# hi-paris/Prosody-Control-French-TTS

Hardware: AMD Instinct MI355X
Metric: audio-seconds/sec prosody+align throughput, 16 kHz French (higher is better)
Workload: dtype fp16-resid16 (MFMA legs) + f64 (F0 / LUFS)

## Files before the change

prosody-control-french-tts_amd/csrc/pce_ctx.hip:

```cpp
#include "pce_internal.h"
#include <cstdlib>
#include <cstring>
#include <cstdarg>

int pce_fail(pce_ctx *ctx, int code, const char *fmt, ...)
{
    char buf[512];
    va_list ap; va_start(ap, fmt);
    vsnprintf(buf, sizeof buf, fmt, ap);
    va_end(ap);
    if (ctx) ctx->err = buf;
    return code;
}

KernelTimer::KernelTimer(pce_ctx *ctx, int kid, hipStream_t on, double work_flops) : c(ctx), id(kid), s(on ? on : ctx->stream), flops(work_flops)
{
    if (!c->prof) return;
    auto take = [&]() -> hipEvent_t {
        if (!c->ev_pool.empty()) { hipEvent_t e = c->ev_pool.back(); c->ev_pool.pop_back(); return e; }
        hipEvent_t e = nullptr;
        if (hipEventCreate(&e) != hipSuccess) return nullptr;
        return e;
    };
    a = take(); b = take();
// ... 73 lines not shown
        return nullptr;
    }
    if (device < 0 || device >= n) {
        if (err && errlen) snprintf(err, errlen, "device %d out of range (0..%d)", device, n - 1);
        return nullptr;
    }
    if ((e = hipSetDevice(device)) != hipSuccess) return fail("hipSetDevice", e);
    hipDeviceProp_t prop;
    if ((e = hipGetDeviceProperties(&prop, device)) != hipSuccess) return fail("hipGetDeviceProperties", e);
    pce_ctx *c = new (std::nothrow) pce_ctx();
    if (!c) { if (err && errlen) snprintf(err, errlen, "out of host memory"); return nullptr; }
    c->device = device;
    c->cu_count = prop.multiProcessorCount;
    if (stream) { c->stream = (hipStream_t)stream; c->own_stream = false; }
    else {
        if ((e = hipStreamCreateWithFlags(&c->stream, hipStreamNonBlocking)) != hipSuccess) { delete c; return fail("hipStreamCreate", e); }
        c->own_stream = true;
    }
    c->no_side = getenv("PCE_NO_AUX") != nullptr;
    c->stft_two_fft = getenv("PCE_STFT_TWO_FFT") != nullptr;
    c->generic_median = getenv("PCE_ALIGN_GENERIC_MEDIAN") != nullptr;
    c->gemm_flat = !(getenv("PCE_GEMM_FLAT") && atoi(getenv("PCE_GEMM_FLAT")) == 0);
    if (const char *re = getenv("PCE_RESID_EPILOGUE")) c->resid_epilogue = atoi(re) == 0 ? 0 : atoi(re) == 2 ? 2 : 1;
    c->en_cpb = getenv("PCE_EN_CPB") ? atoi(getenv("PCE_EN_CPB")) : 0;
    c->gemm_skinny = !(getenv("PCE_GEMM_SKINNY") && atoi(getenv("PCE_GEMM_SKINNY")) == 0);
    c->self_rows = !(getenv("PCE_SELF_ROWS") && atoi(getenv("PCE_SELF_ROWS")) == 0);
    c->xattn_absorb = !(getenv("PCE_XATTN_ABSORB") && atoi(getenv("PCE_XATTN_ABSORB")) == 0);
    {
        const char *ops = getenv("PCE_WHISPER_OPERANDS");
        if (ops && *ops && strcmp(ops, "bf16") && strcmp(ops, "fp16") && strcmp(ops, "fp16-resid16")) {
            if (err && errlen) snprintf(err, errlen, "PCE_WHISPER_OPERANDS=%s: bf16, fp16 or fp16-resid16", ops);
            if (c->own_stream) (void)hipStreamDestroy(c->stream);
            delete c;
            return nullptr;
        }
        c->whisper_ops = (ops && !strcmp(ops, "bf16")) ? 0 : (ops && !strcmp(ops, "fp16")) ? 1 : 2;
        c->resid16 = c->whisper_ops == 2;
    }
    c->pitch_refine_praat = getenv("PCE_PITCH_REFINE") && !strcmp(getenv("PCE_PITCH_REFINE"), "praat");
    if (getenv("PCE_DTW_TRACE_MB") && atoll(getenv("PCE_DTW_TRACE_MB")) > 0) c->dtw_trace_budget = (size_t)atoll(getenv("PCE_DTW_TRACE_MB")) << 20;
    int prio_least = 0, prio_greatest = 0;
    (void)hipDeviceGetStreamPriorityRange(&prio_least, &prio_greatest);
    for (int si = 0; si < pce_ctx::SIDE_COUNT; si++) {
        pce_ctx::Side &sd = c->side[si];
        const int prio = si == pce_ctx::SIDE_STFT ? prio_least : 0;
        if ((e = hipStreamCreateWithPriority(&sd.s, hipStreamNonBlocking, prio)) != hipSuccess) { delete c; return fail("hipStreamCreate", e); }
// ... 204 lines not shown
```

prosody-control-french-tts_amd/csrc/pce_internal.h:

```cpp
#pragma once
#include <hip/hip_runtime.h>
#include <cstdint>
#include <cstdio>
#include <cstring>
#include <string>
#include <vector>
#include "pce.h"

#if defined(__HIP_DEVICE_COMPILE__)
#define PCE_NO_PK_F32 __attribute__((target("no-packed-fp32-ops")))
#else
#define PCE_NO_PK_F32
#endif

struct DevBuf {
    void *p = nullptr;
    size_t cap = 0;
    DevBuf() = default;
    DevBuf(const DevBuf &) = delete;
    DevBuf &operator=(const DevBuf &) = delete;
    DevBuf &operator=(DevBuf &&o) noexcept {
        if (this != &o) { release(); p = o.p; cap = o.cap; o.p = nullptr; o.cap = 0; }
        return *this;
    }
// ... 14 lines not shown
struct SliceCache {
    std::vector<pce_slice> v;
    bool valid = false;
    bool same(const pce_slice *s, int32_t n) const {
        return valid && (size_t)n == v.size() && (n == 0 || memcmp(v.data(), s, sizeof(pce_slice) * (size_t)n) == 0);
    }
    void store(const pce_slice *s, int32_t n) { v.assign(s, s + n); valid = true; }
    void drop() { valid = false; v.clear(); }
};

struct pce_ctx {
    int device = 0;
    hipStream_t stream = nullptr;
    bool own_stream = false;
    enum { SIDE_TAIL = 0, SIDE_LUFS = 1, SIDE_STFT = 2, SIDE_COUNT = 3 };
    struct Side { hipStream_t s = nullptr; hipEvent_t fork = nullptr, join = nullptr; bool pending = false; } side[SIDE_COUNT];
    bool no_side = false;
    bool generic_median = false;
    bool pitch_refine_praat = false;
    bool gemm_few_rows = false;
    bool gemm_skinny = true;
    bool gemm_flat = true;
    int resid_epilogue = 1;
    bool stft_two_fft = false;
    std::string err;
    int cu_count = 0;

    DevBuf pcm_own;
    const int16_t *d_pcm = nullptr;
    DevBuf d_clip_off;
    std::vector<int64_t> clip_off;
    int32_t n_clips = 0;
    int32_t rate = 0;

    int en_cpb = 0;
    DevBuf en_work, en_out;
    SliceCache en_cache;
    int64_t en_n_work = 0;
    int32_t en_n = -1;

    DevBuf lu_meta, lu_chunks, lu_blocks, lu_pow, lu_state_end, lu_state_init, lu_energy, lu_zbuf, lu_out, lu_en_work, lu_en_acc;
    SliceCache lu_cache;
    int64_t lu_n_chunks = 0, lu_n_blocks = 0, lu_n_energy_work = 0;
    double lu_coef[13] = {0};
    int32_t lu_n = -1;
    int32_t lu_meter_rate = 0;
// ... 116 lines not shown
```

prosody-control-french-tts_amd/csrc/pce_whisper_impl.inc:

```
#include "pce_internal.h"
#include "pce_wave.h"
#include <algorithm>
#include <cmath>
#include <cstdlib>
#include <type_traits>

#define pce_logmel_run PCE_WFN(pce_logmel_run)
#define pce_logmel_run_at PCE_WFN(pce_logmel_run_at)
#define pce_logmel_fetch PCE_WFN(pce_logmel_fetch)
#define pce_whisper_load PCE_WFN(pce_whisper_load)
#define pce_whisper_encode_run PCE_WFN(pce_whisper_encode_run)
#define pce_whisper_encode_fetch PCE_WFN(pce_whisper_encode_fetch)
#define pce_selftest_attention PCE_WFN(pce_selftest_attention)
#define pce_selftest_attention_ragged PCE_WFN(pce_selftest_attention_ragged)
#define pce_selftest_attn1 PCE_WFN(pce_selftest_attn1)
#define pce_selftest_gemm PCE_WFN(pce_selftest_gemm)
#define pce_selftest_gemm_resid PCE_WFN(pce_selftest_gemm_resid)
#define pce_whisper_decoder_load PCE_WFN(pce_whisper_decoder_load)
#define pce_whisper_align_run PCE_WFN(pce_whisper_align_run)
#define pce_whisper_align_fetch PCE_WFN(pce_whisper_align_fetch)
#define pce_whisper_align_shape PCE_WFN(pce_whisper_align_shape)
#define pce_whisper_align_paths_enqueue PCE_WFN(pce_whisper_align_paths_enqueue)
#define pce_whisper_align_paths_wait PCE_WFN(pce_whisper_align_paths_wait)
#define pce_whisper_sample_keys PCE_WFN(pce_whisper_sample_keys)
// ... 12 lines not shown
                                          const uint8_t *vocab_mask, const pce_whisper_decode_opts *opts, int32_t *next_tokens,
                                          float *next_logprobs, float *probe_prob);
void pce_whisper_free(pce_ctx *c);

namespace {

typedef PCE_OP_T op_t;
typedef __attribute__((ext_vector_type(8))) op_t opx8;
typedef __attribute__((ext_vector_type(4))) float f32x4;

template <class T> struct MfmaOf;
template <> struct MfmaOf<__bf16> {
    typedef __attribute__((ext_vector_type(8))) __bf16 v8;
    static __device__ __forceinline__ f32x4 m16(v8 a, v8 b, f32x4 c) { return __builtin_amdgcn_mfma_f32_16x16x32_bf16(a, b, c, 0, 0, 0); }
};
template <> struct MfmaOf<_Float16> {
    typedef __attribute__((ext_vector_type(8))) _Float16 v8;
    static __device__ __forceinline__ f32x4 m16(v8 a, v8 b, f32x4 c) { return __builtin_amdgcn_mfma_f32_16x16x32_f16(a, b, c, 0, 0, 0); }
};
__device__ __forceinline__ f32x4 mfma16(opx8 a, opx8 b, f32x4 c) { return MfmaOf<op_t>::m16(a, b, c); }

constexpr int W_NFFT = 400, W_HOP = 160, W_BINS = 201, W_FRAMES = 3000, W_SAMPLES = 480000;
constexpr int W_CTX = 1500;
constexpr double W_PI = 3.14159265358979323846;

struct MelTables {
    const float2 *w16;
    const float2 *w400;
    const float2 *w25;
    const float *window;
    const int *mel_lo;
    const int *mel_n;
    const int *mel_off;
    const float *mel_w;
    int mel_total;
};

__device__ __forceinline__ unsigned int f32_order_key(float f)
{
    const unsigned int b = __float_as_uint(f);
    return (b & 0x80000000u) ? ~b : (b | 0x80000000u);
}
__device__ __forceinline__ float f32_from_key(unsigned int k)
{
    return __uint_as_float((k & 0x80000000u) ? (k & 0x7FFFFFFFu) : ~k);
}
// ... 93 lines not shown
                ob[b * (LM_G + 1) + j] = lg;
                vmax = fmaxf(vmax, lg);
            }
        }
        __builtin_amdgcn_fence(__ATOMIC_ACQ_REL, "wavefront"); __builtin_amdgcn_wave_barrier();
      }
      __builtin_amdgcn_fence(__ATOMIC_ACQ_REL, "wavefront"); __builtin_amdgcn_wave_barrier();
      if (!scan && (f_begin + gi * LM_G) * W_HOP - W_NFFT / 2 < len) {
          const int64_t f0 = gi * LM_G;
          const int nj = (int)min<int64_t>(LM_G, n_fr - f0);
          for (int idx = lane; idx < n_mels * LM_G; idx += 64) {
              const int b = idx / LM_G, j = idx - b * LM_G;
              if (j < nj) logspec[((int64_t)clip * n_mels + b) * W_FRAMES + f0 + j] = ob[b * (LM_G + 1) + j];
          }
      }
      __builtin_amdgcn_fence(__ATOMIC_ACQ_REL, "wavefront"); __builtin_amdgcn_wave_barrier();
    }
    vmax = wave_xor_max(vmax);
    if (lane == 0) atomicMax(clip_max + clip, f32_order_key(vmax));
}

__global__ __launch_bounds__(256) void k_logmel_norm(const float *__restrict__ logspec, const unsigned int *__restrict__ clip_max, int n_mels,
                                                    const int64_t *__restrict__ clip_off, const int64_t *__restrict__ frame0, int clip0,
                                                    op_t *__restrict__ out_tm, float *__restrict__ out_f32)
{
    __shared__ float tile[64][65];
    const int clip = clip0 + blockIdx.z, f0 = blockIdx.x * 64, b0 = blockIdx.y * 64;
    const float floor_v = f32_from_key(clip_max[clip]) - 8.0f;
    const int64_t full = clip_off[clip + 1] - clip_off[clip];
    const int64_t len = frame0 ? full : min<int64_t>(full, (int64_t)W_SAMPLES), f_begin = frame0 ? frame0[clip] : 0;
    const float pad_v = (fmaxf(log10f(fmaxf(0.f, 1e-10f)), floor_v) + 4.0f) / 4.0f;
    const int tx = threadIdx.x & 63, ty = threadIdx.x >> 6;
    const bool padded = (f_begin + f0 + tx) * W_HOP - W_NFFT / 2 >= len;
    for (int r = ty; r < 64; r += 4) {
        const int b = b0 + r, f = f0 + tx;
        if (b < n_mels && f < W_FRAMES) {
            const float v = padded ? pad_v : (fmaxf(logspec[((int64_t)clip * n_mels + b) * W_FRAMES + f], floor_v) + 4.0f) / 4.0f;
            if (out_f32) out_f32[(int64_t)b * W_FRAMES + f] = v;
            tile[r][tx] = v;
        }
    }
    if (!out_tm) return;
    __syncthreads();
    for (int r = ty; r < 64; r += 4) {
        const int f = f0 + r, b = b0 + tx;
        if (b < n_mels && f < W_FRAMES) out_tm[((int64_t)clip * (W_FRAMES + 2) + f + 1) * n_mels + b] = (op_t)tile[tx][r];
    }
}

enum { EPI_BF16 = 0, EPI_GELU_BF16 = 1, EPI_GELU_POS_F32 = 2, EPI_RESID_F32 = 3, EPI_QKV = 4, EPI_F32 = 5 };
constexpr int AT_SP = 1536;
constexpr int G_BM = 128, G_BN = 128, G_BK = 64;

constexpr float GELU_C = 0.70710678118654752440f * 1.2011224087864498f;
constexpr float GELU_P = 0.3275911f / 1.2011224087864498f;
__device__ __forceinline__ float gelu_exact(float x)
{
    const float zp = fabsf(x) * GELU_C;
    const float t = __builtin_amdgcn_rcpf(fmaf(zp, GELU_P, 1.0f));
    const float e = __builtin_amdgcn_exp2f(zp * -zp);
    const float poly = fmaf(t, fmaf(t, fmaf(t, fmaf(t, 1.061405429f, -1.453152027f), 1.421413741f), -0.284496736f), 0.254829592f);
    const float erf_abs = fmaf(-(t * poly), e, 1.0f);
    const float h = 0.5f * x;
    return fmaf(fabsf(h), erf_abs, h);
}
__device__ __forceinline__ void gelu_exact8(float (&x)[8])
{
    float zp[8], t[8], e[8], poly[8], h[8];
#pragma unroll
    for (int i = 0; i < 8; i++) zp[i] = fabsf(x[i]) * GELU_C;
#pragma unroll
    for (int i = 0; i < 8; i++) t[i] = __builtin_amdgcn_rcpf(fmaf(zp[i], GELU_P, 1.0f));
#pragma unroll
    for (int i = 0; i < 8; i++) e[i] = __builtin_amdgcn_exp2f(zp[i] * -zp[i]);
#pragma unroll
// ... 26 lines not shown
        const int r0 = wv * 16 + i * 8;
        const int row = r0 + (lane >> 3);
        const int c = swz_chunk(row, lane & 7);
        int gr = row0 + row; if (gr > row_max) gr = row_max;
        const op_t *src = G + (int64_t)gr * ld + k0 + c * 8;
        __builtin_amdgcn_global_load_lds((const __attribute__((address_space(1))) void *)src,
                                         (__attribute__((address_space(3))) void *)(lds_tile + r0 * G_BK), 16, 0, 0);
    }
}

template <int EPI>
__device__ __forceinline__ void gemm_fetch_bias(const float *__restrict__ bias, int n0, int tid, float (&bv)[8], float &bv_col)
{
    constexpr bool OUT_BF16 = (EPI == EPI_BF16 || EPI == EPI_GELU_BF16 || EPI == EPI_QKV);
    const int cx0 = OUT_BF16 ? (tid & 15) * 8 : (tid & 31) * 4;
#pragma unroll
    for (int e = 0; e < 8; e++) bv[e] = (bias && e < (OUT_BF16 ? 8 : 4)) ? bias[n0 + cx0 + e] : 0.f;
    bv_col = (EPI == EPI_QKV && bias) ? bias[n0 + (tid & 127)] : 0.f;
}

template <int EPI>
__device__ __forceinline__ void gemm_store_tile(const float *tile, int tid, int m0, int n0, int M, int N, const float (&bv)[8], float bv_col,
                                                void *__restrict__ Cv, int64_t ldc, int64_t cbase, const float *__restrict__ pos, int pos_T,
                                                int v_col0, int vt_sp)
{
    if (EPI == EPI_QKV && n0 >= v_col0) {
        op_t *vt = reinterpret_cast<op_t *>(const_cast<float *>(pos));
        const int dmodel = N - v_col0, S = pos_T;
        const int cc = tid & 127, rg = tid >> 7;
        const int n = n0 + cc - v_col0, head = n >> 6, dd = n & 63;
        const float bv = bv_col;
#pragma unroll
        for (int p = 0; p < 4; p++) {
            const int row = rg * 8 + 32 * p;
#pragma unroll
            for (int hf = 0; hf < 2; hf++) {
                const int m = m0 + row + 4 * hf;
                if (m >= M) continue;
                const int clip = m / S, t = m - clip * S;
                typedef __attribute__((ext_vector_type(4))) op_t opx4;
                opx4 o;
#pragma unroll
                for (int e = 0; e < 4; e++) o[e] = (op_t)(tile[(row + 4 * hf + e) * G_TLD + cc] + bv);
                *reinterpret_cast<opx4 *>(vt + (((int64_t)clip * (dmodel >> 6) + head) * 64 + dd) * vt_sp + t) = o;
            }
        }
    } else if (EPI == EPI_BF16 || EPI == EPI_GELU_BF16 || EPI == EPI_QKV) {
// ... 12 lines not shown
                o[e] = (op_t)(EPI == EPI_GELU_BF16 ? gelu_exact(t) : t);
            }
            __builtin_nontemporal_store(o, reinterpret_cast<opx8 *>(reinterpret_cast<op_t *>(Cv) + cbase + (int64_t)(m0 + row) * ldc + n0 + cx));
        }
    } else {
        const int cx = (tid & 31) * 4, ry = tid >> 5;
        float4 oldv[8];
        if (EPI == EPI_RESID_F32) {
#pragma unroll
            for (int p = 0; p < 8; p++) {
                const int row = ry + 16 * p;
                oldv[p] = m0 + row < M ? *reinterpret_cast<const float4 *>(reinterpret_cast<const float *>(Cv) + cbase + (int64_t)(m0 + row) * ldc + n0 + cx)
                                       : make_float4(0.f, 0.f, 0.f, 0.f);
            }
        }
#pragma unroll
        for (int p = 0; p < 8; p++) {
            const int row = ry + 16 * p;
            if (m0 + row >= M) continue;
            const float4 v = *reinterpret_cast<const float4 *>(&tile[row * G_TLD + cx]);
            float4 *dst = reinterpret_cast<float4 *>(reinterpret_cast<float *>(Cv) + cbase + (int64_t)(m0 + row) * ldc + n0 + cx);
            float4 o;
            if (EPI == EPI_GELU_POS_F32) {
                const float4 pe = *reinterpret_cast<const float4 *>(pos + (int64_t)((m0 + row) % pos_T) * N + n0 + cx);
                o = make_float4(gelu_exact(v.x + bv[0]) + pe.x, gelu_exact(v.y + bv[1]) + pe.y, gelu_exact(v.z + bv[2]) + pe.z,
                                gelu_exact(v.w + bv[3]) + pe.w);
            } else {
                const float4 old = EPI == EPI_RESID_F32 ? oldv[p] : make_float4(0.f, 0.f, 0.f, 0.f);
                o = make_float4(old.x + v.x + bv[0], old.y + v.y + bv[1], old.z + v.z + bv[2], old.w + v.w + bv[3]);
            }
            *dst = o;
        }
    }
}

template <int EPI, int G_STAGES = 2>
__global__ __launch_bounds__(G_THREADS, G_STAGES == 2 ? 4 : 2) void k_gemm_bf16(const op_t *__restrict__ A, int64_t lda, int64_t a_batch,
                                                        const op_t *__restrict__ B, int M, int N, int K,
                                                        const float *__restrict__ bias, void *__restrict__ Cv, int64_t ldc, int64_t c_batch,
                                                        const float *__restrict__ pos, int pos_T, int v_col0, int vt_sp, int sn_tiles, int sm_tiles)
{
    constexpr int SMEM_ELEMS = (G_STAGES * 2 * G_BM * G_BK * 2 > G_BM * G_TLD * 4 ? G_STAGES * 2 * G_BM * G_BK : G_BM * G_TLD * 2);
    __shared__ __attribute__((aligned(1024))) op_t smem[SMEM_ELEMS];
    const int tid = threadIdx.x, lane = tid & 63, wv = tid >> 6;
    const int wr = wv >> 2, wc = wv & 3;
    const int tiles_n = (int)gridDim.x, tiles_m_pad = (int)gridDim.y;
    int lin = (int)blockIdx.y * tiles_n + (int)blockIdx.x;
    const int total = tiles_n * tiles_m_pad;
    if ((total & 7) == 0) lin = (lin & 7) * (total >> 3) + (lin >> 3);
    int m0, n0;
    {
        const int per = sm_tiles * sn_tiles, sup = lin / per, r = lin - sup * per;
        const int n_sn = tiles_n / sn_tiles;
        const int tm = (sup / n_sn) * sm_tiles + r / sn_tiles, tn = (sup % n_sn) * sn_tiles + r % sn_tiles;
        m0 = tm * G_BM; n0 = tn * G_BN;
        if (m0 >= M) return;
    }
    float bv[8]; float bv_col;
    gemm_fetch_bias<EPI>(bias, n0, tid, bv, bv_col);
    A += (int64_t)blockIdx.z * a_batch;
    f32x4 acc[4][2];
#pragma unroll
    for (int i = 0; i < 4; i++)
#pragma unroll
        for (int j = 0; j < 2; j++) acc[i][j] = f32x4{0.f, 0.f, 0.f, 0.f};
    const int fr = lane & 15, fq = lane >> 4;
    const int nk = K / G_BK;
    constexpr int STAGE = 2 * G_BM * G_BK;
#pragma unroll
    for (int t = 0; t < G_STAGES - 1; t++) {
        const int tt = t < nk ? t : nk - 1;
        stage_tile(A, lda, m0, M - 1, tt * G_BK, smem + t * STAGE, wv, lane);
        stage_tile(B, K, n0, N - 1, tt * G_BK, smem + t * STAGE + G_BM * G_BK, wv, lane);
    }
    for (int kt = 0; kt < nk; kt++) {
        const op_t *sA = smem + (kt % G_STAGES) * STAGE, *sB = sA + G_BM * G_BK;
        __builtin_amdgcn_s_waitcnt(0x0F70 | (((4 * (G_STAGES - 2)) >> 4) << 14) | ((4 * (G_STAGES - 2)) & 15));
        __builtin_amdgcn_s_barrier();
        if (G_STAGES > 2 || kt + G_STAGES - 1 < nk) {
// ... 12 lines not shown
            }
#pragma unroll
            for (int j = 0; j < 2; j++) {
                const int row = wc * 32 + j * 16 + fr;
                b[j] = *reinterpret_cast<const opx8 *>(&sB[row * G_BK + swz_chunk(row, (kk >> 3) + fq) * 8]);
            }
#pragma unroll
            for (int i = 0; i < 4; i++)
#pragma unroll
                for (int j = 0; j < 2; j++) acc[i][j] = mfma16(a[i], b[j], acc[i][j]);
        }
    }
    if (G_STAGES > 2) asm volatile("s_waitcnt vmcnt(0)" ::: "memory");
    __builtin_amdgcn_s_barrier();
    float *tile = reinterpret_cast<float *>(smem);
#pragma unroll
    for (int i = 0; i < 4; i++)
#pragma unroll
        for (int j = 0; j < 2; j++)
#pragma unroll
            for (int r = 0; r < 4; r++)
                tile[(wr * 64 + i * 16 + fq * 4 + r) * G_TLD + wc * 32 + j * 16 + fr] = acc[i][j][r];
    __syncthreads();
    gemm_store_tile<EPI>(tile, tid, m0, n0, M, N, bv, bv_col, Cv, ldc, (int64_t)blockIdx.z * c_batch, pos, pos_T, v_col0, vt_sp);
}

constexpr int S_BM = 64, S_BN = 32, S_KC = 256, S_THREADS = 256, S_NBUF = 3;
constexpr int S_BUF = (S_BM + S_BN) * S_KC;
constexpr int S_LDS = S_NBUF * S_BUF * 2;
__device__ __forceinline__ int swz512(int row, int chunk) { return chunk ^ (row & 15); }
template <int EPI>
__global__ __launch_bounds__(S_THREADS) void k_gemm_skinny(const op_t *__restrict__ A, int64_t lda, const op_t *__restrict__ B, int M, int N, int K,
                                                           const float *__restrict__ bias, void *__restrict__ Cv, int64_t ldc)
{
    extern __shared__ __attribute__((aligned(1024))) op_t sk[];
    const int tid = threadIdx.x, lane = tid & 63, wv = __builtin_amdgcn_readfirstlane(tid >> 6);
    const int fr = lane & 15, fq = lane >> 4;
    const int n0 = blockIdx.x * S_BN, m0 = blockIdx.y * S_BM;
    const int nk = K / S_KC;
    auto stage = [&](int kc, int buf) {
        op_t *dst = sk + buf * S_BUF;
#pragma unroll
        for (int i = 0; i < 12; i++) {
            const int inst = wv + 4 * i, row = inst * 2 + (lane >> 5);
            const int c = swz512(row, lane & 31);
            const op_t *src;
            if (row < S_BM) { int gr = m0 + row; if (gr > M - 1) gr = M - 1; src = A + (int64_t)gr * lda + kc * S_KC + c * 8; }
// ... 1153 lines not shown
    auto hz_to_mel = [&](double f) { return f >= min_log_hz ? min_log_mel + std::log(f / min_log_hz) / logstep : f / f_sp; };
    auto mel_to_hz = [&](double m) { return m >= min_log_mel ? min_log_hz * std::exp(logstep * (m - min_log_mel)) : f_sp * m; };
    std::vector<double> mel_f((size_t)n_mels + 2), fft_f(W_BINS);
    const double m_lo = hz_to_mel(0.0), m_hi = hz_to_mel(sr / 2);
    for (int i = 0; i < n_mels + 2; i++) mel_f[(size_t)i] = mel_to_hz(m_lo + (m_hi - m_lo) * i / (n_mels + 1));
    for (int k = 0; k < W_BINS; k++) fft_f[(size_t)k] = (sr / 2) * k / (W_BINS - 1);
    dense.assign((size_t)n_mels * W_BINS, 0.f);
    for (int i = 0; i < n_mels; i++) {
        const double enorm = 2.0 / (mel_f[(size_t)i + 2] - mel_f[(size_t)i]);
        for (int k = 0; k < W_BINS; k++) {
            const double lower = -(mel_f[(size_t)i] - fft_f[(size_t)k]) / (mel_f[(size_t)i + 1] - mel_f[(size_t)i]);
            const double upper = (mel_f[(size_t)i + 2] - fft_f[(size_t)k]) / (mel_f[(size_t)i + 2] - mel_f[(size_t)i + 1]);
            const double w = std::max(0.0, std::min(lower, upper));
            dense[(size_t)i * W_BINS + k] = (float)(w * enorm);
        }
    }
}

struct WhisperState {
    pce_whisper_dims dims{};
    bool loaded = false;
    DevBuf tables, logspec, clipmax, mel_tm, mel_start, mel_stage, w_bf16, w_f32, pos;
    bool mel_windowed = false;
    DevBuf c1_out, resid, resid16, ln_out, qkv, vt, attn, hidden, final_out, enc_tab, delta, delta2;
    size_t vt_elems_zeroed = 0;
    std::vector<int> al_tab_host, al_tok_host, al_heads_host;
    size_t mel_tm_zero_cap = 0, c1_zero_cap = 0, dvt_zero_cap = 0; int mel_tm_zero_nm = 0, c1_zero_d = 0;
    pce_whisper_text_dims tdims{};
    bool dec_loaded = false;
    DevBuf dw_bf16, dw_f32, d_tok_emb, d_pos_emb;
    DevBuf d_tab, d_tokens, d_resid, d_ln, d_qk, d_vt, d_attn, d_q, d_hidden, d_enc_bf16, d_aw, d_cost, d_trace, d_pi, d_pj, d_pl, d_heads;
    int enc_bf16_clips = -1;
    DevBuf g_emb_bf16, g_xk, g_xvt, g_last, g_lastln, g_logits, g_mask, g_next, g_keys;
    DevBuf g_lang;
    DevBuf g_wkT, g_qp, g_upart, g_mlpart;
    int g_keys_n = 0;
    int g_xkv_clips = -1;
    DevBuf g_sv;
    DevBuf g_sk, g_svt, g_c_resid, g_c_ln, g_c_qkv, g_c_attn, g_c_q, g_c_hidden, g_c_tab, g_loop;
    std::vector<int> g_cache_tok;
    int g_cache_len = -1, g_cache_n = -1;
    std::vector<int> g_cache_lens;
    struct DLayer { size_t ln1_w, ln1_b, qkv_w, qkv_b, out_w, out_b, lnx_w, lnx_b, xq_w, xq_b, xkv_w, xkv_b, xout_w, xout_b,
                    ln2_w, ln2_b, m1_w, m1_b, m2_w, m2_b; };
    std::vector<DLayer> dlayers;
    size_t dln_w = 0, dln_b = 0;
// ... 109 lines not shown
enum GemmKernel { GK_AUTO = 0, GK_SKINNY = 1, GK_WIDE = 2, GK_128 = 3, GK_128_DEEP = 4 };
struct GemmShape { int M, N, K; int64_t lda; int batch; int v_col0; };
template <int EPI> static bool gemm_fits(int kind, const GemmShape &s)
{
    switch (kind) {
    case GK_SKINNY:
        return (EPI == EPI_BF16 || EPI == EPI_GELU_BF16 || EPI == EPI_RESID_F32) && s.batch == 1 && s.M <= 1024 && s.N <= 4096 && s.N % S_BN == 0 &&
               s.K % S_KC == 0 && s.lda % 8 == 0;
    case GK_WIDE: return s.N % W_BN == 0 && s.K % W_BK == 0 && (EPI != EPI_QKV || s.v_col0 % W_BN == 0);
    case GK_128: case GK_128_DEEP: return s.N % G_BN == 0 && s.K % G_BK == 0 && (EPI != EPI_QKV || s.v_col0 % G_BN == 0);
    default: return false;
    }
}
template <int EPI> static int gemm_choose(const pce_ctx *c, const GemmShape &s)
{
    if (c->gemm_skinny && c->gemm_few_rows && gemm_fits<EPI>(GK_SKINNY, s)) return GK_SKINNY;
    if (gemm_fits<EPI>(GK_WIDE, s) && s.N >= 1536 && !(EPI == EPI_F32 && (int64_t)s.M * s.batch <= 1024))
        return GK_WIDE;
    if ((int64_t)s.M * s.batch <= 1024 && s.K >= 4 * G_BK) return GK_128_DEEP;
    return GK_128;
}
template <int EPI>
static void launch_gemm_kernel(pce_ctx *c, int kind, const op_t *A, int64_t lda, int64_t a_batch, const op_t *B, int M, int N, int K, const float *bias,
                               void *C, int64_t ldc, int64_t c_batch, int batch, const float *pos, int pos_T, int v_col0, int vt_sp)
{
    if constexpr (EPI == EPI_BF16 || EPI == EPI_GELU_BF16 || EPI == EPI_RESID_F32) {
        if (kind == GK_SKINNY) {
            KernelTimer kt(c, PCE_K_GEMM_SKINNY, nullptr, 2.0 * M * (double)N * K);
            hipLaunchKernelGGL((k_gemm_skinny<EPI>), dim3((unsigned)(N / S_BN), (unsigned)div_up(M, S_BM)), dim3(S_THREADS), S_LDS, c->stream,
                               A, lda, B, M, N, K, bias, C, ldc);
            return;
        }
    }
    if (kind == GK_WIDE) {
        const int wt = N / W_BN;
        int wsn = 1;
        for (int cand : {4, 3, 2}) if (wt % cand == 0) { wsn = cand; break; }
        const int wsm = 16;
        dim3 wgrid((unsigned)wt, (unsigned)(div_up(M, G_BM * wsm) * wsm), (unsigned)batch);
        KernelTimer kt(c, PCE_K_GEMM_WIDE, nullptr, 2.0 * M * (double)N * K * batch);
        hipLaunchKernelGGL((k_gemm_wide<EPI>), wgrid, dim3(G_THREADS), 0, c->stream, A, lda, a_batch, B, M, N, K, bias, C, ldc, c_batch, pos, pos_T,
                           v_col0, vt_sp, wsn, wsm);
        return;
    }
    const int tiles_n = N / G_BN;
    int sn = 1;
    for (int cand : {8, 6, 4, 3, 2}) if (tiles_n % cand == 0) { sn = cand; break; }
    const int sm = 16;
    dim3 grid((unsigned)tiles_n, (unsigned)(div_up(M, G_BM * sm) * sm), (unsigned)batch);
    KernelTimer kt(c, PCE_K_GEMM128, nullptr, 2.0 * M * (double)N * K * batch);
    if (kind == GK_128_DEEP)
        hipLaunchKernelGGL((k_gemm_bf16<EPI, 4>), grid, dim3(G_THREADS), 0, c->stream, A, lda, a_batch, B, M, N, K, bias, C, ldc, c_batch, pos, pos_T,
                           v_col0, vt_sp, sn, sm);
    else
        hipLaunchKernelGGL((k_gemm_bf16<EPI>), grid, dim3(G_THREADS), 0, c->stream, A, lda, a_batch, B, M, N, K, bias, C, ldc, c_batch, pos, pos_T,
                           v_col0, vt_sp, sn, sm);
}
template <int EPI>
void launch_gemm(pce_ctx *c, const op_t *A, int64_t lda, int64_t a_batch, const op_t *B, int M, int N, int K, const float *bias,
                 void *C, int64_t ldc, int64_t c_batch, int batch, const float *pos = nullptr, int pos_T = 1, int v_col0 = 0,
                 int vt_sp = AT_SP)
{
    const int kind = gemm_choose<EPI>(c, GemmShape{M, N, K, lda, batch, v_col0});
    launch_gemm_kernel<EPI>(c, kind, A, lda, a_batch, B, M, N, K, bias, C, ldc, c_batch, batch, pos, pos_T, v_col0, vt_sp);
}

template <class OUT>
static void launch_layernorm(pce_ctx *c, const float *x, const float *w, const float *b, int64_t rows, int d, OUT *out, float eps = 1e-5f,
                             float *out2 = nullptr, int round_in16 = 0, op_t *in16_out = nullptr)
{
    const dim3 grid((unsigned)div_up(rows, 4)), block(256);
    if (d <= 1280) hipLaunchKernelGGL((k_layernorm<OUT, 5>), grid, block, 0, c->stream, x, w, b, rows, d, out, eps, out2, round_in16, in16_out);
    else hipLaunchKernelGGL((k_layernorm<OUT, 8>), grid, block, 0, c->stream, x, w, b, rows, d, out, eps, out2, round_in16, in16_out);
}
template <class OUT, class RIN, class ROUT>
static void launch_add_layernorm(pce_ctx *c, const RIN *resid_in, ROUT *resid_out, const op_t *delta, const op_t *delta2, int write_resid, const float *w,
                                 const float *b, int64_t rows, int d, OUT *out, float eps, op_t *out_bf16)
{
    const dim3 grid((unsigned)div_up(rows, 4)), block(256);
    if (d <= 1280)
        hipLaunchKernelGGL((k_add_layernorm<OUT, RIN, ROUT, 5>), grid, block, 0, c->stream, resid_in, resid_out, delta, delta2, write_resid, w, b, rows, d, out, eps, out_bf16);
    else
        hipLaunchKernelGGL((k_add_layernorm<OUT, RIN, ROUT, 8>), grid, block, 0, c->stream, resid_in, resid_out, delta, delta2, write_resid, w, b, rows, d, out, eps, out_bf16);
}

template <class OUT>
static void launch_add_layernorm0(pce_ctx *c, const op_t *x, const float *w, const float *b, int64_t rows, int d, OUT *out, float eps, op_t *out_bf16)
// ... 99 lines not shown

static int logmel_run_impl(pce_ctx *c, int32_t n_mels, const int64_t *start_frames);
int pce_logmel_run(pce_ctx *c, int32_t n_mels) { return logmel_run_impl(c, n_mels, nullptr); }
int pce_logmel_run_at(pce_ctx *c, int32_t n_mels, const int64_t *start_frames)
{
    if (!start_frames) return PCE_E_INVALID;
    return logmel_run_impl(c, n_mels, start_frames);
}
static int logmel_run_impl(pce_ctx *c, int32_t n_mels, const int64_t *start_frames)
{
    if (!c) return PCE_E_INVALID;
    if (!c->d_pcm) return pce_fail(c, PCE_E_STATE, "no batch uploaded");
    if (c->rate != 16000) return pce_fail(c, PCE_E_INVALID, "log-mel needs 16 kHz audio (got %d Hz): resample on the host first", c->rate);
    if (n_mels <= 0 || n_mels > 128) return pce_fail(c, PCE_E_INVALID, "n_mels %d out of range", n_mels);
    PCE_HIP(c, hipSetDevice(c->device));
    WhisperState *w = ws_of(c);
    int rc = mel_setup(c, w, n_mels);
    if (rc) return rc;
    const int32_t n = c->n_clips;
    const size_t tm_elems = (size_t)n * (W_FRAMES + 2) * (size_t)n_mels + 512;
    PCE_HIP(c, w->logspec.reserve(sizeof(float) * (size_t)n * (size_t)n_mels * W_FRAMES));
    PCE_HIP(c, w->clipmax.reserve(sizeof(unsigned int) * (size_t)n));
    PCE_HIP(c, w->mel_tm.reserve(sizeof(op_t) * tm_elems));
    PCE_HIP(c, hipMemsetAsync(w->clipmax.p, 0, sizeof(unsigned int) * (size_t)n, c->stream));
    if (w->mel_tm.cap != w->mel_tm_zero_cap || w->mel_tm_zero_nm != n_mels) {
        PCE_HIP(c, hipMemsetAsync(w->mel_tm.p, 0, w->mel_tm.cap, c->stream));
        w->mel_tm_zero_cap = w->mel_tm.cap; w->mel_tm_zero_nm = n_mels;
    }
    constexpr int LM_G = 16;
    const size_t lm_lds = sizeof(float) * 4 * (size_t)n_mels * (LM_G + 1);
    const int64_t *d_start = nullptr;
    if (start_frames) {
        int64_t longest = 0;
        for (int32_t i = 0; i < n; i++) {
            const int64_t len = c->clip_off[(size_t)i + 1] - c->clip_off[(size_t)i];
            if (start_frames[i] < 0 || start_frames[i] * W_HOP > len) return pce_fail(c, PCE_E_INVALID, "clip %d: window start %lld frames is past the audio", i, (long long)start_frames[i]);
            longest = std::max(longest, len);
        }
        PCE_HIP(c, w->mel_start.reserve(sizeof(int64_t) * (size_t)(n > 0 ? n : 1)));
        PCE_HIP(c, hipMemcpyAsync(w->mel_start.p, start_frames, sizeof(int64_t) * (size_t)n, hipMemcpyHostToDevice, c->stream));
        PCE_HIP(c, hipStreamSynchronize(c->stream));
        d_start = w->mel_start.as<int64_t>();
        if (n > 0) {
            const int64_t scan_frames = (longest + W_NFFT / 2) / W_HOP + 1;
            hipLaunchKernelGGL(k_logmel_frames<LM_G>, dim3((unsigned)std::min<int64_t>(div_up(scan_frames, 4 * LM_G), 4096), (unsigned)n), dim3(256), lm_lds, c->stream, c->d_pcm,
                               c->d_clip_off.as<int64_t>(), (int)n_mels, w->mt, w->logspec.as<float>(), w->clipmax.as<unsigned int>(), d_start, 1);
        }
    }
    {
        KernelTimer t(c, PCE_K_LOGMEL);
        hipLaunchKernelGGL(k_logmel_frames<LM_G>, dim3((unsigned)div_up(W_FRAMES, 4 * LM_G), (unsigned)n), dim3(256), lm_lds, c->stream, c->d_pcm,
                           c->d_clip_off.as<int64_t>(), (int)n_mels, w->mt, w->logspec.as<float>(), w->clipmax.as<unsigned int>(), d_start, 0);
    }
    {
        KernelTimer t(c, PCE_K_LOGMEL_NORM);
        hipLaunchKernelGGL(k_logmel_norm, dim3(div_up(W_FRAMES, 64), div_up(n_mels, 64), (unsigned)n), dim3(256), 0, c->stream,
                           w->logspec.as<float>(), w->clipmax.as<unsigned int>(), (int)n_mels, c->d_clip_off.as<int64_t>(), d_start, 0, w->mel_tm.as<op_t>(), (float *)nullptr);
    }
    PCE_HIP(c, hipGetLastError());
    w->n_clips_mel = n;
    w->mel_windowed = start_frames != nullptr;
    return PCE_OK;
}

int pce_logmel_fetch(pce_ctx *c, int32_t clip, float *out)
{
    if (!c || !out) return PCE_E_INVALID;
    WhisperState *w = ws_of(c);
    if (w->n_clips_mel < 0) return pce_fail(c, PCE_E_STATE, "pce_logmel_fetch before pce_logmel_run");
    if (clip < 0 || clip >= w->n_clips_mel) return pce_fail(c, PCE_E_INVALID, "clip out of range");
    const size_t per = (size_t)w->mel_nmels * W_FRAMES;
    PCE_HIP(c, hipSetDevice(c->device));
    PCE_HIP(c, w->mel_stage.reserve(sizeof(float) * per + 64));
    hipLaunchKernelGGL(k_logmel_norm, dim3(div_up(W_FRAMES, 64), div_up(w->mel_nmels, 64), 1), dim3(256), 0, c->stream, w->logspec.as<float>(),
                       w->clipmax.as<unsigned int>(), (int)w->mel_nmels, c->d_clip_off.as<int64_t>(), w->mel_windowed ? w->mel_start.as<int64_t>() : (const int64_t *)nullptr,
                       (int)clip, (op_t *)nullptr, w->mel_stage.as<float>());
    PCE_HIP(c, hipGetLastError());
    PCE_HIP(c, hipMemcpyAsync(out, w->mel_stage.p, sizeof(float) * per, hipMemcpyDeviceToHost, c->stream));
    PCE_HIP(c, hipStreamSynchronize(c->stream));
    pce_profile_collect(c);
    return PCE_OK;
}

int pce_whisper_load(pce_ctx *c, const pce_whisper_dims *dims, const float *weights, int64_t n_floats)
{
    if (!c || !dims || !weights) return PCE_E_INVALID;
    const int d = dims->n_state, L = dims->n_layer, nm = dims->n_mels;
    if (d <= 0 || d % 128 || dims->n_head * 64 != d || L <= 0 || dims->n_ctx != W_CTX || nm <= 0 || nm > 128 || (nm % 8))
        return pce_fail(c, PCE_E_LIMIT, "unsupported encoder dims (need n_state %% 128 == 0, head size 64, n_ctx 1500, n_mels %% 8 == 0)");
    if (d > LN_D_MAX) return pce_fail(c, PCE_E_LIMIT, "encoder with n_state %d: the LayerNorm kernels hold at most %d", d, LN_D_MAX);
    if (c->gemm_flat && d % F_T == 0 && 4 * d > F_N_MAX)
        return pce_fail(c, PCE_E_LIMIT, "encoder with n_state %d: the persistent GEMM's fc1 holds 4 n_state <= %d (PCE_GEMM_FLAT=0 at pce_create runs it on the "
                                        "tiled kernels)", d, F_N_MAX);
    const int64_t per_layer = 2LL * d + 4LL * d * d + 3LL * d + 2LL * d + 8LL * d * d + 5LL * d;
    const int64_t expect = (int64_t)d * nm * 3 + d + 3LL * d * d + d + L * per_layer + 2LL * d;
    if (n_floats != expect) return pce_fail(c, PCE_E_INVALID, "weight blob has %lld floats, expected %lld", (long long)n_floats, (long long)expect);
    PCE_HIP(c, hipSetDevice(c->device));
    WhisperState *w = ws_of(c);
    { const int rc = lds_optins(c, w); if (rc) return rc; }
// ... 88 lines not shown
        if (w->vt.cap != before || w->vt_elems_zeroed < vt_elems) {
            PCE_HIP(c, hipMemsetAsync(w->vt.p, 0, sizeof(op_t) * vt_elems, c->stream));
            w->vt_elems_zeroed = vt_elems;
        }
    }
    PCE_HIP(c, w->attn.reserve(sizeof(op_t) * (size_t)M * d));
    PCE_HIP(c, w->hidden.reserve(sizeof(op_t) * (size_t)M * 4 * d));
    PCE_HIP(c, w->final_out.reserve(sizeof(float) * (size_t)M * d));
    const op_t *Wb = w->w_bf16.as<op_t>();
    const float *Wf = w->w_f32.as<float>();
    if (w->enc_tab_clips != n) {
        std::vector<int> tab((size_t)2 * n);
        for (int i = 0; i < n; i++) { tab[(size_t)i] = i * W_CTX; tab[(size_t)n + i] = W_CTX; }
        PCE_HIP(c, w->enc_tab.reserve(sizeof(int) * tab.size()));
        PCE_HIP(c, hipMemcpyAsync(w->enc_tab.p, tab.data(), sizeof(int) * tab.size(), hipMemcpyHostToDevice, c->stream));
        PCE_HIP(c, hipStreamSynchronize(c->stream));
        w->enc_tab_clips = n;
    }
    KernelTimer t(c, PCE_K_WHISPER_ENC);
    if (w->c1_out.cap != w->c1_zero_cap || w->c1_zero_d != d) {
        PCE_HIP(c, hipMemsetAsync(w->c1_out.p, 0, w->c1_out.cap, c->stream));
        w->c1_zero_cap = w->c1_out.cap; w->c1_zero_d = d;
    }
    launch_gemm<EPI_GELU_BF16>(c, w->mel_tm.as<op_t>(), nm, (int64_t)(W_FRAMES + 2) * nm, Wb + w->c1_w, W_FRAMES, d, K1p, Wf + w->c1_b,
                               w->c1_out.as<op_t>() + d, d, (int64_t)(W_FRAMES + 2) * d, n);
    launch_gemm<EPI_GELU_POS_F32>(c, w->c1_out.as<op_t>(), 2 * (int64_t)d, (int64_t)(W_FRAMES + 2) * d, Wb + w->c2_w, W_CTX, d, 3 * d,
                                  Wf + w->c2_b, w->resid.as<float>(), d, (int64_t)W_CTX * d, n, w->pos.as<float>(), W_CTX);
    const bool flat = c->gemm_flat && d % F_T == 0 && gemm_flat_offsets_fit(M, 4 * d, 4 * d, 4 * d, 0, 0) &&
                      gemm_flat_offsets_fit(M, d, d, 0, W_CTX, AT_SP);
    if (flat) PCE_HIP(c, w->d_enc_bf16.reserve(sizeof(op_t) * (size_t)M * d + 4096));
    const bool resid16 = flat && c->resid16 && PCE_OP_INDEX == 1;
    if (resid16) PCE_HIP(c, w->resid16.reserve(sizeof(op_t) * (size_t)M * d));
    const bool fused = resid16 && c->resid_epilogue != 0, fused_out = fused && c->resid_epilogue == 1;
    if (flat && !fused_out) PCE_HIP(c, w->delta.reserve(sizeof(op_t) * (size_t)M * d));
    if (flat && !fused) PCE_HIP(c, w->delta2.reserve(sizeof(op_t) * (size_t)M * d));
    auto add_ln = [&](size_t w_off, size_t b_off, bool mid, bool last, bool first_layer) {
        KernelTimer kt(c, PCE_K_ADD_LAYERNORM);
        const op_t *d2 = mid ? nullptr : w->delta2.as<op_t>();
        float *r32 = w->resid.as<float>(); op_t *r16 = w->resid16.as<op_t>();
        const float *lw = Wf + w_off, *lb = Wf + b_off;
        const int wr = mid ? 0 : 1;
        if (fused && mid && !fused_out) {
            launch_add_layernorm<op_t, op_t, op_t>(c, r16, r16, w->delta.as<op_t>(), nullptr, 1, lw, lb, M, d, w->ln_out.as<op_t>(), 1e-5f, nullptr);
            return;
        }
        if (fused) {
            if (last) launch_add_layernorm0<float>(c, r16, lw, lb, M, d, w->final_out.as<float>(), 1e-5f, w->d_enc_bf16.as<op_t>());
            else launch_add_layernorm0<op_t>(c, r16, lw, lb, M, d, w->ln_out.as<op_t>(), 1e-5f, nullptr);
            return;
        }
// ... 78 lines not shown
```

Measured before the change: 20570.

## Skip conv stem GEMM tiles over zero-padded mel frames and fill from repeated row

Whisper pads each clip's mel to 3000 frames, so conv1/conv2 rows past the clip's audio see only constant padding and produce identical outputs. The mel-normalise kernel now records per clip which 128-row tiles fall entirely in that region. The stem GEMMs skip those tiles, conv2 saves one representative accumulator row, and a small fill kernel writes GELU+bias+positional embedding for the skipped rows. This removes stem MFMA work for short clips. It adds a launch, swizzle changes and a correctness dependence on the padded rows really being identical.

```diff
diff --git a/prosody-control-french-tts_amd/csrc/pce_ctx.hip b/prosody-control-french-tts_amd/csrc/pce_ctx.hip
--- a/prosody-control-french-tts_amd/csrc/pce_ctx.hip
+++ b/prosody-control-french-tts_amd/csrc/pce_ctx.hip
@@ -119,6 +119,7 @@
     c->generic_median = getenv("PCE_ALIGN_GENERIC_MEDIAN") != nullptr;
     c->gemm_flat = !(getenv("PCE_GEMM_FLAT") && atoi(getenv("PCE_GEMM_FLAT")) == 0);
     if (const char *re = getenv("PCE_RESID_EPILOGUE")) c->resid_epilogue = atoi(re) == 0 ? 0 : atoi(re) == 2 ? 2 : 1;
+    c->stem_skip = !(getenv("PCE_STEM_SKIP") && atoi(getenv("PCE_STEM_SKIP")) == 0);
     c->en_cpb = getenv("PCE_EN_CPB") ? atoi(getenv("PCE_EN_CPB")) : 0;
     c->gemm_skinny = !(getenv("PCE_GEMM_SKINNY") && atoi(getenv("PCE_GEMM_SKINNY")) == 0);
     c->self_rows = !(getenv("PCE_SELF_ROWS") && atoi(getenv("PCE_SELF_ROWS")) == 0);
diff --git a/prosody-control-french-tts_amd/csrc/pce_internal.h b/prosody-control-french-tts_amd/csrc/pce_internal.h
--- a/prosody-control-french-tts_amd/csrc/pce_internal.h
+++ b/prosody-control-french-tts_amd/csrc/pce_internal.h
@@ -60,6 +60,7 @@
     bool gemm_skinny = true;
     bool gemm_flat = true;
     int resid_epilogue = 1;
+    bool stem_skip = true;
     bool stft_two_fft = false;
     std::string err;
     int cu_count = 0;
diff --git a/prosody-control-french-tts_amd/csrc/pce_whisper_impl.inc b/prosody-control-french-tts_amd/csrc/pce_whisper_impl.inc
--- a/prosody-control-french-tts_amd/csrc/pce_whisper_impl.inc
+++ b/prosody-control-french-tts_amd/csrc/pce_whisper_impl.inc
@@ -58,6 +58,23 @@
 
 constexpr int W_NFFT = 400, W_HOP = 160, W_BINS = 201, W_FRAMES = 3000, W_SAMPLES = 480000;
 constexpr int W_CTX = 1500;
+constexpr int ST_TILE = 128;
+constexpr int ST_C2_LAST = (W_CTX - 1) / ST_TILE;
+constexpr int ST_C1_KEEP = (2 * ST_TILE * ST_C2_LAST - 1) / ST_TILE;
+static_assert(ST_TILE * ST_C2_LAST < W_CTX - 1, "the last conv2 tile must hold a repeated row in front of row 1499");
+struct GemmSkip {
+    const int2 *tiles;
+    float *rep; int rep_row;
+    int64_t skipped_rows;
+};
+__host__ __device__ inline int stem_first_skipped_tile(int64_t len, int64_t f_begin)
+{
+    const int64_t p64 = (len + W_NFFT / 2 + W_HOP - 1) / W_HOP - f_begin;
+    const int P = (int)(p64 < 0 ? 0 : p64 > W_FRAMES ? W_FRAMES : p64);
+    const int r2 = (P + 3) / 2;
+    const int s = (r2 + ST_TILE - 1) / ST_TILE;
+    return s < ST_C2_LAST ? s : ST_C2_LAST;
+}
 constexpr double W_PI = 3.14159265358979323846;
 
 struct MelTables {
@@ -197,13 +214,19 @@
 
 __global__ __launch_bounds__(256) void k_logmel_norm(const float *__restrict__ logspec, const unsigned int *__restrict__ clip_max, int n_mels,
                                                     const int64_t *__restrict__ clip_off, const int64_t *__restrict__ frame0, int clip0,
-                                                    op_t *__restrict__ out_tm, float *__restrict__ out_f32)
+                                                    op_t *__restrict__ out_tm, float *__restrict__ out_f32,
+                                                    int2 *__restrict__ skip_c1, int2 *__restrict__ skip_c2)
 {
     __shared__ float tile[64][65];
     const int clip = clip0 + blockIdx.z, f0 = blockIdx.x * 64, b0 = blockIdx.y * 64;
     const float floor_v = f32_from_key(clip_max[clip]) - 8.0f;
     const int64_t full = clip_off[clip + 1] - clip_off[clip];
     const int64_t len = frame0 ? full : min<int64_t>(full, (int64_t)W_SAMPLES), f_begin = frame0 ? frame0[clip] : 0;
+    if (skip_c1 && blockIdx.x == 0 && blockIdx.y == 0 && threadIdx.x == 0) {
+        const int s = stem_first_skipped_tile(len, f_begin);
+        skip_c2[clip] = make_int2(s, ST_C2_LAST - 1);
+        skip_c1[clip] = s < ST_C2_LAST ? make_int2(2 * s, ST_C1_KEEP - 1) : make_int2(1, 0);
+    }
     const float pad_v = (fmaxf(log10f(fmaxf(0.f, 1e-10f)), floor_v) + 4.0f) / 4.0f;
     const int tx = threadIdx.x & 63, ty = threadIdx.x >> 6;
     const bool padded = (f_begin + f0 + tx) * W_HOP - W_NFFT / 2 >= len;
@@ -226,6 +249,7 @@
 enum { EPI_BF16 = 0, EPI_GELU_BF16 = 1, EPI_GELU_POS_F32 = 2, EPI_RESID_F32 = 3, EPI_QKV = 4, EPI_F32 = 5 };
 constexpr int AT_SP = 1536;
 constexpr int G_BM = 128, G_BN = 128, G_BK = 64;
+static_assert(G_BM == ST_TILE, "the stem's skip ranges count k_gemm_bf16 row tiles");
 
 constexpr float GELU_C = 0.70710678118654752440f * 1.2011224087864498f;
 constexpr float GELU_P = 0.3275911f / 1.2011224087864498f;
@@ -298,7 +322,7 @@
 template <int EPI>
 __device__ __forceinline__ void gemm_store_tile(const float *tile, int tid, int m0, int n0, int M, int N, const float (&bv)[8], float bv_col,
                                                 void *__restrict__ Cv, int64_t ldc, int64_t cbase, const float *__restrict__ pos, int pos_T,
-                                                int v_col0, int vt_sp)
+                                                int v_col0, int vt_sp, float *__restrict__ rep = nullptr, int rep_row = 0)
 {
     if (EPI == EPI_QKV && n0 >= v_col0) {
         op_t *vt = reinterpret_cast<op_t *>(const_cast<float *>(pos));
@@ -357,6 +381,7 @@
             float4 *dst = reinterpret_cast<float4 *>(reinterpret_cast<float *>(Cv) + cbase + (int64_t)(m0 + row) * ldc + n0 + cx);
             float4 o;
             if (EPI == EPI_GELU_POS_F32) {
+                if (rep && m0 + row == rep_row) *reinterpret_cast<float4 *>(rep + n0 + cx) = v;
                 const float4 pe = *reinterpret_cast<const float4 *>(pos + (int64_t)((m0 + row) % pos_T) * N + n0 + cx);
                 o = make_float4(gelu_exact(v.x + bv[0]) + pe.x, gelu_exact(v.y + bv[1]) + pe.y, gelu_exact(v.z + bv[2]) + pe.z,
                                 gelu_exact(v.w + bv[3]) + pe.w);
@@ -373,7 +398,8 @@
 __global__ __launch_bounds__(G_THREADS, G_STAGES == 2 ? 4 : 2) void k_gemm_bf16(const op_t *__restrict__ A, int64_t lda, int64_t a_batch,
                                                         const op_t *__restrict__ B, int M, int N, int K,
                                                         const float *__restrict__ bias, void *__restrict__ Cv, int64_t ldc, int64_t c_batch,
-                                                        const float *__restrict__ pos, int pos_T, int v_col0, int vt_sp, int sn_tiles, int sm_tiles)
+                                                        const float *__restrict__ pos, int pos_T, int v_col0, int vt_sp, int sn_tiles, int sm_tiles,
+                                                        GemmSkip skip)
 {
     constexpr int SMEM_ELEMS = (G_STAGES * 2 * G_BM * G_BK * 2 > G_BM * G_TLD * 4 ? G_STAGES * 2 * G_BM * G_BK : G_BM * G_TLD * 2);
     __shared__ __attribute__((aligned(1024))) op_t smem[SMEM_ELEMS];
@@ -382,7 +408,7 @@
     const int tiles_n = (int)gridDim.x, tiles_m_pad = (int)gridDim.y;
     int lin = (int)blockIdx.y * tiles_n + (int)blockIdx.x;
     const int total = tiles_n * tiles_m_pad;
-    if ((total & 7) == 0) lin = (lin & 7) * (total >> 3) + (lin >> 3);
+    if ((total & 7) == 0) lin = (((lin & 7) + (skip.tiles ? (int)blockIdx.z : 0)) & 7) * (total >> 3) + (lin >> 3);
     int m0, n0;
     {
         const int per = sm_tiles * sn_tiles, sup = lin / per, r = lin - sup * per;
@@ -390,6 +416,10 @@
         const int tm = (sup / n_sn) * sm_tiles + r / sn_tiles, tn = (sup % n_sn) * sn_tiles + r % sn_tiles;
         m0 = tm * G_BM; n0 = tn * G_BN;
         if (m0 >= M) return;
+        if (skip.tiles) {
+            const int2 sk = skip.tiles[blockIdx.z];
+            if (tm >= sk.x && tm <= sk.y) return;
+        }
     }
     float bv[8]; float bv_col;
     gemm_fetch_bias<EPI>(bias, n0, tid, bv, bv_col);
@@ -448,7 +478,28 @@
             for (int r = 0; r < 4; r++)
                 tile[(wr * 64 + i * 16 + fq * 4 + r) * G_TLD + wc * 32 + j * 16 + fr] = acc[i][j][r];
     __syncthreads();
-    gemm_store_tile<EPI>(tile, tid, m0, n0, M, N, bv, bv_col, Cv, ldc, (int64_t)blockIdx.z * c_batch, pos, pos_T, v_col0, vt_sp);
+    gemm_store_tile<EPI>(tile, tid, m0, n0, M, N, bv, bv_col, Cv, ldc, (int64_t)blockIdx.z * c_batch, pos, pos_T, v_col0, vt_sp,
+                         skip.rep ? skip.rep + (int64_t)blockIdx.z * N : nullptr, skip.rep_row);
+}
+
+constexpr int SF_ROWS = 16;
+static_assert(ST_TILE % SF_ROWS == 0, "a fill workgroup must not straddle a tile boundary");
+__global__ __launch_bounds__(256) void k_stem_fill(const int2 *__restrict__ tiles, const float *__restrict__ rep, const float *__restrict__ bias,
+                                                   const float *__restrict__ pos , int d , float *__restrict__ out )
+{
+    const int clip = blockIdx.y, t0 = blockIdx.x * SF_ROWS;
+    if (t0 < tiles[clip].x * ST_TILE || t0 >= ST_C2_LAST * ST_TILE) return;
+    const int d4 = d >> 2;
+    const float *acc = rep + (int64_t)clip * d;
+    float *dst = out + ((int64_t)clip * W_CTX + t0) * d;
+    const float *pe0 = pos + (int64_t)t0 * d;
+    for (int i = threadIdx.x; i < SF_ROWS * d4; i += 256) {
+        const int cx = (i % d4) * 4;
+        const float4 v = *reinterpret_cast<const float4 *>(acc + cx), b = *reinterpret_cast<const float4 *>(bias + cx);
+        const float4 pe = *reinterpret_cast<const float4 *>(pe0 + (int64_t)i * 4);
+        const float4 o = make_float4(gelu_exact(v.x + b.x) + pe.x, gelu_exact(v.y + b.y) + pe.y, gelu_exact(v.z + b.z) + pe.z, gelu_exact(v.w + b.w) + pe.w);
+        *reinterpret_cast<float4 *>(dst + (int64_t)i * 4) = o;
+    }
 }
 
 constexpr int S_BM = 64, S_BN = 32, S_KC = 256, S_THREADS = 256, S_NBUF = 3;
@@ -1648,6 +1699,8 @@
     bool loaded = false;
     DevBuf tables, logspec, clipmax, mel_tm, mel_start, mel_stage, w_bf16, w_f32, pos;
     bool mel_windowed = false;
+    int64_t stem_tiles_c1 = 0, stem_tiles_c2 = 0;
+    DevBuf stem_skip, stem_rep;
     DevBuf c1_out, resid, resid16, ln_out, qkv, vt, attn, hidden, final_out, enc_tab, delta, delta2;
     size_t vt_elems_zeroed = 0;
     std::vector<int> al_tab_host, al_tok_host, al_heads_host;
@@ -1803,7 +1856,8 @@
 }
 template <int EPI>
 static void launch_gemm_kernel(pce_ctx *c, int kind, const op_t *A, int64_t lda, int64_t a_batch, const op_t *B, int M, int N, int K, const float *bias,
-                               void *C, int64_t ldc, int64_t c_batch, int batch, const float *pos, int pos_T, int v_col0, int vt_sp)
+                               void *C, int64_t ldc, int64_t c_batch, int batch, const float *pos, int pos_T, int v_col0, int vt_sp,
+                               const GemmSkip &skip = GemmSkip{nullptr, nullptr, 0, 0})
 {
     if constexpr (EPI == EPI_BF16 || EPI == EPI_GELU_BF16 || EPI == EPI_RESID_F32) {
         if (kind == GK_SKINNY) {
@@ -1829,21 +1883,22 @@
     for (int cand : {8, 6, 4, 3, 2}) if (tiles_n % cand == 0) { sn = cand; break; }
     const int sm = 16;
     dim3 grid((unsigned)tiles_n, (unsigned)(div_up(M, G_BM * sm) * sm), (unsigned)batch);
-    KernelTimer kt(c, PCE_K_GEMM128, nullptr, 2.0 * M * (double)N * K * batch);
+    KernelTimer kt(c, PCE_K_GEMM128, nullptr, 2.0 * ((double)M * batch - (double)skip.skipped_rows) * N * K);
     if (kind == GK_128_DEEP)
         hipLaunchKernelGGL((k_gemm_bf16<EPI, 4>), grid, dim3(G_THREADS), 0, c->stream, A, lda, a_batch, B, M, N, K, bias, C, ldc, c_batch, pos, pos_T,
-                           v_col0, vt_sp, sn, sm);
+                           v_col0, vt_sp, sn, sm, GemmSkip{nullptr, nullptr, 0, 0});
     else
         hipLaunchKernelGGL((k_gemm_bf16<EPI>), grid, dim3(G_THREADS), 0, c->stream, A, lda, a_batch, B, M, N, K, bias, C, ldc, c_batch, pos, pos_T,
-                           v_col0, vt_sp, sn, sm);
+                           v_col0, vt_sp, sn, sm, skip);
 }
 template <int EPI>
 void launch_gemm(pce_ctx *c, const op_t *A, int64_t lda, int64_t a_batch, const op_t *B, int M, int N, int K, const float *bias,
                  void *C, int64_t ldc, int64_t c_batch, int batch, const float *pos = nullptr, int pos_T = 1, int v_col0 = 0,
-                 int vt_sp = AT_SP)
+                 int vt_sp = AT_SP, const GemmSkip *skip = nullptr)
 {
     const int kind = gemm_choose<EPI>(c, GemmShape{M, N, K, lda, batch, v_col0});
-    launch_gemm_kernel<EPI>(c, kind, A, lda, a_batch, B, M, N, K, bias, C, ldc, c_batch, batch, pos, pos_T, v_col0, vt_sp);
+    if (skip && kind == GK_128) launch_gemm_kernel<EPI>(c, kind, A, lda, a_batch, B, M, N, K, bias, C, ldc, c_batch, batch, pos, pos_T, v_col0, vt_sp, *skip);
+    else launch_gemm_kernel<EPI>(c, kind, A, lda, a_batch, B, M, N, K, bias, C, ldc, c_batch, batch, pos, pos_T, v_col0, vt_sp);
 }
 
 template <class OUT>
@@ -1989,6 +2044,13 @@
     PCE_HIP(c, w->logspec.reserve(sizeof(float) * (size_t)n * (size_t)n_mels * W_FRAMES));
     PCE_HIP(c, w->clipmax.reserve(sizeof(unsigned int) * (size_t)n));
     PCE_HIP(c, w->mel_tm.reserve(sizeof(op_t) * tm_elems));
+    PCE_HIP(c, w->stem_skip.reserve(sizeof(int2) * 2 * (size_t)(n > 0 ? n : 1)));
+    w->stem_tiles_c1 = w->stem_tiles_c2 = 0;
+    for (int32_t i = 0; i < n; i++) {
+        const int64_t full = c->clip_off[(size_t)i + 1] - c->clip_off[(size_t)i];
+        const int s = stem_first_skipped_tile(start_frames ? full : std::min<int64_t>(full, W_SAMPLES), start_frames ? start_frames[i] : 0);
+        if (s < ST_C2_LAST) { w->stem_tiles_c2 += ST_C2_LAST - s; w->stem_tiles_c1 += ST_C1_KEEP - 2 * s; }
+    }
     PCE_HIP(c, hipMemsetAsync(w->clipmax.p, 0, sizeof(unsigned int) * (size_t)n, c->stream));
     if (w->mel_tm.cap != w->mel_tm_zero_cap || w->mel_tm_zero_nm != n_mels) {
         PCE_HIP(c, hipMemsetAsync(w->mel_tm.p, 0, w->mel_tm.cap, c->stream));
@@ -2022,7 +2084,8 @@
     {
         KernelTimer t(c, PCE_K_LOGMEL_NORM);
         hipLaunchKernelGGL(k_logmel_norm, dim3(div_up(W_FRAMES, 64), div_up(n_mels, 64), (unsigned)n), dim3(256), 0, c->stream,
-                           w->logspec.as<float>(), w->clipmax.as<unsigned int>(), (int)n_mels, c->d_clip_off.as<int64_t>(), d_start, 0, w->mel_tm.as<op_t>(), (float *)nullptr);
+                           w->logspec.as<float>(), w->clipmax.as<unsigned int>(), (int)n_mels, c->d_clip_off.as<int64_t>(), d_start, 0, w->mel_tm.as<op_t>(), (float *)nullptr,
+                           w->stem_skip.as<int2>(), w->stem_skip.as<int2>() + n);
     }
     PCE_HIP(c, hipGetLastError());
     w->n_clips_mel = n;
@@ -2041,7 +2104,7 @@
     PCE_HIP(c, w->mel_stage.reserve(sizeof(float) * per + 64));
     hipLaunchKernelGGL(k_logmel_norm, dim3(div_up(W_FRAMES, 64), div_up(w->mel_nmels, 64), 1), dim3(256), 0, c->stream, w->logspec.as<float>(),
                        w->clipmax.as<unsigned int>(), (int)w->mel_nmels, c->d_clip_off.as<int64_t>(), w->mel_windowed ? w->mel_start.as<int64_t>() : (const int64_t *)nullptr,
-                       (int)clip, (op_t *)nullptr, w->mel_stage.as<float>());
+                       (int)clip, (op_t *)nullptr, w->mel_stage.as<float>(), (int2 *)nullptr, (int2 *)nullptr);
     PCE_HIP(c, hipGetLastError());
     PCE_HIP(c, hipMemcpyAsync(out, w->mel_stage.p, sizeof(float) * per, hipMemcpyDeviceToHost, c->stream));
     PCE_HIP(c, hipStreamSynchronize(c->stream));
@@ -2176,10 +2239,22 @@
         PCE_HIP(c, hipMemsetAsync(w->c1_out.p, 0, w->c1_out.cap, c->stream));
         w->c1_zero_cap = w->c1_out.cap; w->c1_zero_d = d;
     }
+    const bool stem_skip = c->stem_skip && w->stem_tiles_c2 > 0 && gemm_choose<EPI_GELU_BF16>(c, GemmShape{W_FRAMES, d, K1p, nm, n, 0}) == GK_128 &&
+                           gemm_choose<EPI_GELU_POS_F32>(c, GemmShape{W_CTX, d, 3 * d, 2 * (int64_t)d, n, 0}) == GK_128;
+    GemmSkip skip1{nullptr, nullptr, 0, 0}, skip2 = skip1;
+    if (stem_skip) {
+        PCE_HIP(c, w->stem_rep.reserve(sizeof(float) * (size_t)n * d));
+        const int2 *sk = w->stem_skip.as<int2>();
+        skip1 = GemmSkip{sk, nullptr, 0, w->stem_tiles_c1 * ST_TILE};
+        skip2 = GemmSkip{sk + n, w->stem_rep.as<float>(), ST_TILE * ST_C2_LAST, w->stem_tiles_c2 * ST_TILE};
+    }
     launch_gemm<EPI_GELU_BF16>(c, w->mel_tm.as<op_t>(), nm, (int64_t)(W_FRAMES + 2) * nm, Wb + w->c1_w, W_FRAMES, d, K1p, Wf + w->c1_b,
-                               w->c1_out.as<op_t>() + d, d, (int64_t)(W_FRAMES + 2) * d, n);
+                               w->c1_out.as<op_t>() + d, d, (int64_t)(W_FRAMES + 2) * d, n, nullptr, 1, 0, AT_SP, stem_skip ? &skip1 : nullptr);
     launch_gemm<EPI_GELU_POS_F32>(c, w->c1_out.as<op_t>(), 2 * (int64_t)d, (int64_t)(W_FRAMES + 2) * d, Wb + w->c2_w, W_CTX, d, 3 * d,
-                                  Wf + w->c2_b, w->resid.as<float>(), d, (int64_t)W_CTX * d, n, w->pos.as<float>(), W_CTX);
+                                  Wf + w->c2_b, w->resid.as<float>(), d, (int64_t)W_CTX * d, n, w->pos.as<float>(), W_CTX, 0, AT_SP, stem_skip ? &skip2 : nullptr);
+    if (stem_skip)
+        hipLaunchKernelGGL(k_stem_fill, dim3((unsigned)(ST_TILE * ST_C2_LAST / SF_ROWS), (unsigned)n), dim3(256), 0, c->stream, skip2.tiles, w->stem_rep.as<float>(),
+                           Wf + w->c2_b, w->pos.as<float>(), d, w->resid.as<float>());
     const bool flat = c->gemm_flat && d % F_T == 0 && gemm_flat_offsets_fit(M, 4 * d, 4 * d, 4 * d, 0, 0) &&
                       gemm_flat_offsets_fit(M, d, d, 0, W_CTX, AT_SP);
     if (flat) PCE_HIP(c, w->d_enc_bf16.reserve(sizeof(op_t) * (size_t)M * d + 4096));
```

New measurement: 20830 (median of 6 runs). +1.3%, better.
